# ahtamjidi/3PRE

Measured on AMD Instinct MI355X. Metric: EKF steps/sec (predict+RANSAC+update) at N=500 landmarks; P-update %MFMA peak, higher is better.
Workload: dtype f32

## Files before the change

3pre_amd/_lib.py:

```python
import ctypes as C
import os

import numpy as np

try:
    import torch
except Exception:
    torch = None

_HERE = os.path.dirname(os.path.abspath(__file__))
LIB_PATH = os.environ.get("PRE3_LIB") or os.path.join(_HERE, "lib", "libpre3.so")

if not os.path.exists(LIB_PATH):
    raise ImportError(
        "3pre_amd: %s is missing -- build it with `make -C 3pre_amd/csrc` (or __graft_entry__.build()); "
        "there is no CPU fallback for the HIP path" % LIB_PATH)

lib = C.CDLL(LIB_PATH)
lib.pre3_last_error.restype = C.c_char_p
lib.pre3_version.restype = C.c_char_p
lib.pre3_match_bench_create.restype = C.c_void_p
lib.pre3_match_bench_create_cls.restype = C.c_void_p
lib.pre3_hypothesis_support.argtypes = [C.c_int, C.c_int, C.c_void_p, C.c_void_p, C.c_void_p, C.c_int, C.c_void_p, C.c_int, C.c_void_p, C.c_double, C.c_void_p, C.c_void_p, C.c_void_p]
lib.pre3_step.argtypes = [C.c_void_p, C.c_void_p, C.c_int, C.c_void_p, C.c_void_p, C.c_int, C.c_int, C.c_void_p, C.c_double, C.c_int, C.c_double, C.c_void_p]
# ... 60 lines not shown
lib.pre3_icp.argtypes = [_I, _P, _I, _P, _I, _D, _P, _P, _P, _P, _P, _P]
lib.pre3_icp_limits.argtypes = [_P]
lib.pre3_icp_frames.argtypes = [_P, _P, _I, _D, _P, _P, _P, _P, _P, _P, _P]
lib.pre3_icp_pair_seeded.argtypes = [_P, _P, _D, _U, _U, _I, _D, _P, _P, _P, _P, _P, _P, _P, _P, _P, _P, _P, _P, _P, _P, _P]
lib.pre3_icp_nn_bench.argtypes = [_I, _P, _I, _P, _I, _I, _P]
lib.pre3_icp_cov.argtypes = [_I, _P, _I, _P, _I, _P, _I, _P, _P, _P, _P]
lib.pre3_icp_cov_limits.argtypes = [_P]
lib.pre3_icp_cov_bench.argtypes = [_I, _P, _I, _P, _I, _P, _I, _P, _I, _P]
lib.pre3_predict_icp_pair_seeded.argtypes = [_P, _P, _P, _D, _U, _U, _I, _D, _D, _I, _P, _P, _P, _P, _P, _P]
lib.pre3_icp_pair_cov_seeded.argtypes = [_P, _P, _D, _U, _U, _I, _D, _P, _P, _P, _P, _P, _P, _P, _P, _P, _P, _P, _P, _P, _P, _P, _P, _P, _P, _P]
lib.pre3_epnp.argtypes = [_I, _P, _I, _I, _P, _P, _P]
lib.pre3_pnp_ransac.argtypes = [_I, _P, _I, _I, _P, _P, _I, _P, _D, _P, _P, _P, _P, _P]
lib.pre3_pnp_ransac_seeded.argtypes = [_I, _P, _I, _I, _P, _P, _I, _U, _U, _D, _P, _P, _P, _P, _P, _P]
lib.pre3_pnp_limits.argtypes = [_P]
lib.pre3_vo_pair_pnp_seeded.argtypes = [_P, _P, _D, _U, _U, _P, _I, _P, _P, _P, _P, _P, _P, _P, _P, _P, _P, _P, _P]
lib.pre3_pnp_bench.argtypes = [_I, _P, _I, _I, _P, _P, _I, _U, _U, _D, _I, _P]
lib.pre3_relocalise_seeded.argtypes = [_P, _D, _I, _U, _U, _D, _I, _I, _P, _P, _P, _P]
lib.pre3_reloc_limits.argtypes = [_P]
lib.pre3_pnp_refine.argtypes = [_I, _P, _I, _I, _P, _P, _P, _P, _I, _D, _P]
lib.pre3_pnp_ransac_refined_seeded.argtypes = [_I, _P, _I, _I, _P, _P, _I, _U, _U, _D, _P, _P, _P, _P, _P, _P, _I, _D, _P]
lib.pre3_relocalise_refined_seeded.argtypes = [_P, _D, _I, _U, _U, _D, _I, _I, _I, _D, _I, _P, _P, _P, _P]
lib.pre3_test_downdate.argtypes = [_P, _I, _P, _I]
lib.pre3_test_factor_solve.argtypes = [_P, _I, _P, _P, _P, _I, _I, _P, _P]

F64, F32 = 0, 1
INVDEPTH, CARTESIAN = 0, 1
X_K_K, X_K_KM1 = 0, 1
FAST_MAX_CORNERS, FAST_MAX_ATTEMPTS = 8192, 10


class FastInitResult(C.Structure):
    _fields_ = [("status", C.c_int32), ("attempts", C.c_int32), ("uv", C.c_int32 * 2), ("landmark", C.c_int32), ("pad", C.c_int32), ("rho", C.c_double),
                ("xyz", C.c_double * 3), ("centres", C.c_int32 * 20)]


class Cam(C.Structure):
    _fields_ = [(k, C.c_double) for k in ("f", "Cx", "Cy", "k1", "k2", "nRows", "nCols")]


class Pre3Error(RuntimeError):
    def __init__(self, code, msg):
        super().__init__("libpre3 error %d: %s" % (code, msg))
        self.code = code


def check(rc):
# ... 60 lines not shown
```

3pre_amd/csrc/pre3_api.hip:

```cpp
#include <time.h>
#include <algorithm>
#include <atomic>
#include <immintrin.h>
#include <cmath>
#include <cstdarg>
#include <new>

#include <chrono>
#include "pre3_internal.h"
#include "pre3_test_hooks.h"
#include "pre3_geomdev.h"
#include "pre3_predictu.h"
#include "pre3_predictcv.h"
#include <mutex>
#include "pre3_cholp.h"
#include "pre3_patch.h"
#include "pre3_fast.h"

namespace pre3 {

static thread_local char g_err[512] = "";
void set_error(const char *fmt, ...)
{
    va_list ap; va_start(ap, fmt);
// ... 1534 lines not shown
    c->kt.enabled = false;
    if (mode == 0) c->k9_overlap = false;
    int rc = chol_solve_for_test(c, r_pad, predicted_prior != 0, r);
    c->k9_overlap = ov_was;
    if (rc == PRE3_OK && mode == 1) rc = launch_downdate(c, r, c->W, -1);
    c->kt.enabled = kt_was;
    PRE3_TRY(rc);
    PRE3_TRY(fetch_stats(c));
    if (L_out != nullptr) {
        PRE3_HIP(hipMemcpy(simg.data(), c->Smat, simg.size(), hipMemcpyDeviceToHost));
        for (int i = 0; i < r; ++i)
            for (int j = 0; j < r; ++j) L_out[(size_t)i * r + j] = j <= i ? get(simg, (size_t)i * r_pad + j) : 0.0;
    }
    if (W_out != nullptr) {
        PRE3_HIP(hipMemcpy(wimg.data(), c->W, wimg.size(), hipMemcpyDeviceToHost));
        for (int i = 0; i < r_pad; ++i) {
            for (int j = 0; j < n; ++j) W_out[(size_t)i * (n + 1) + j] = get(wimg, (size_t)i * ldw + j);
            W_out[(size_t)i * (n + 1) + n] = get(wimg, (size_t)i * ldw + c->ld);
        }
    }
    return PRE3_OK;
}

int pre3_match_shard_create_cls(pre3_match_shard **out, int device, int cls, int ND, int K1, const void *L1, int K2_local, const void *L2_local, int k2_offset)
{
    PRE3_CHECK(out != nullptr, PRE3_E_ARG, "pre3_match_shard_create: null output");
    PRE3_TRY(select_device("pre3_match_shard_create", device));
    void *h = match_shard_create(device, cls, ND, K1, L1, K2_local, L2_local, k2_offset);
    if (!h) return PRE3_E_ARG;
    *out = (pre3_match_shard *)h;
    return PRE3_OK;
}
int pre3_match_shard_create(pre3_match_shard **out, int device, int ND, int K1, const uint8_t *L1, int K2_local, const uint8_t *L2_local, int k2_offset)
{
    return pre3_match_shard_create_cls(out, device, 2, ND, K1, L1, K2_local, L2_local, k2_offset);
}
int pre3_match_shard_run(pre3_match_shard *s, void **partial_dev, int *n_doubles) { return s ? match_shard_run(s, partial_dev, n_doubles) : PRE3_E_ARG; }
int pre3_match_shard_merge(pre3_match_shard *s, int G, const void *gathered_dev, double thresh, double *pairs_out, double *score_out, int *M_out)
{
    return s ? match_shard_merge(s, G, gathered_dev, thresh, pairs_out, score_out, M_out) : PRE3_E_ARG;
}
int pre3_match_shard_set_comm(pre3_match_shard *s, pre3_comm *comm) { return s ? match_shard_set_comm(s, comm) : PRE3_E_ARG; }
int pre3_match_shard_match(pre3_match_shard *s, double thresh, double *pairs_out, double *score_out, int *M_out)
{
    return s ? match_shard_match(s, thresh, pairs_out, score_out, M_out) : PRE3_E_ARG;
}
// ... 24 lines not shown
```

3pre_amd/csrc/pre3_geomdev.h:

```cpp
#pragma once
#include "pre3_internal.h"

namespace pre3 {

struct CamD { double f, Cx, Cy, k1, k2, nRows, nCols; };
struct U7 { double v[7]; };
struct VoOut; struct VoPairHeader;
struct PredictUDev { const VoOut *out; const VoPairHeader *hdr; int32_t *err; };
struct VoCov;
struct PnConst {};
struct PnBlock { const double *pn; };
struct PnPair { const VoCov *cov; const VoOut *out; const VoPairHeader *hdr; const double *behind; };
struct IcpCtl;
struct PredictIcpSrc { const VoOut *out; const VoPairHeader *hdr; const VoCov *cov_pair; const IcpCtl *ctl; const double *u_icp, *error; const VoCov *cov_icp;
                       double max_error; int noise; };
struct PredictUIcp { PredictIcpSrc s; int32_t *err; int32_t *taken; };
struct PnIcp { PredictIcpSrc s; const double *behind; };
struct PredictUReloc { const pre3_pnp_result *res; const double *x; int32_t min_support; double *u_out; int32_t *taken_out; };
struct PnReloc { const pre3_pnp_result *res; int32_t min_support; const double *pn; const double *behind; };
struct PredictURelocRef { PredictUReloc b; const pre3_pnp_refine_result *ref; };
struct PnRelocRef { PnReloc b; const pre3_pnp_refine_result *ref; const double *x; int32_t noise; double *pn_out; int32_t *noise_out; };


__device__ inline void d_q2r(const double *q, double *R)
// ... 259 lines not shown
    else active = active && (ic[ii] == 1 && li[ii] == 0);
    const int d = lm_type[ii] == PRE3_INVDEPTH ? 6 : 3;
    const int off = lm_off[ii];
    const int nn = 7 + d;
    double s00 = 0, s01 = 0, s10 = 0, s11 = 0;
    if (active && b < nn) {
        const int ib = b < 7 ? b : off + b - 7;
        const T *prow = P + (size_t)ib * ld;
        double hp0 = 0, hp1 = 0;
#pragma unroll
        for (int a = 0; a < 7; ++a) { double p = (double)prow[a]; hp0 += Hc[14 * ii + a] * p; hp1 += Hc[14 * ii + 7 + a] * p; }
#pragma unroll
        for (int a = 0; a < 6; ++a)
            if (a < d) { double p = (double)prow[off + a]; hp0 += Hl[12 * ii + a] * p; hp1 += Hl[12 * ii + 6 + a] * p; }
        const double h0b = b < 7 ? Hc[14 * ii + b] : Hl[12 * ii + b - 7];
        const double h1b = b < 7 ? Hc[14 * ii + 7 + b] : Hl[12 * ii + 6 + b - 7];
        s00 = hp0 * h0b; s01 = hp0 * h1b; s10 = hp1 * h0b; s11 = hp1 * h1b;
    }
    if (pend_rows > 0 && active) {
        double hc0[7], hc1[7], hl0[6], hl1[6];
#pragma unroll
        for (int a = 0; a < 7; ++a) { hc0[a] = Hc[14 * ii + a]; hc1[a] = Hc[14 * ii + 7 + a]; }
#pragma unroll
        for (int a = 0; a < 6; ++a) { hl0[a] = a < d ? Hl[12 * ii + a] : 0.0; hl1[a] = a < d ? Hl[12 * ii + 6 + a] : 0.0; }
        for (int k = b; k < pend_rows; k += 16) {
            const float *wr = pend_W + (size_t)k * pend_ldw;
            float wp[7], wl[6];
#pragma unroll
            for (int a = 0; a < 7; ++a) wp[a] = wr[a];
#pragma unroll
            for (int a = 0; a < 6; ++a) wl[a] = a < d ? wr[off + a] : 0.f;
            double g0 = 0, g1 = 0;
#pragma unroll
            for (int a = 0; a < 7; ++a) { const double w = (double)wp[a]; g0 += hc0[a] * w; g1 += hc1[a] * w; }
#pragma unroll
            for (int a = 0; a < 6; ++a)
                if (a < d) { const double w = (double)wl[a]; g0 += hl0[a] * w; g1 += hl1[a] * w; }
            s00 -= g0 * g0; s01 -= g0 * g1; s10 -= g1 * g0; s11 -= g1 * g1;
        }
    }
#pragma unroll
    for (int o = 8; o > 0; o >>= 1) {
        s00 += __shfl_xor(s00, o, 16); s01 += __shfl_xor(s01, o, 16);
        s10 += __shfl_xor(s10, o, 16); s11 += __shfl_xor(s11, o, 16);
    }
    if (!valid || b != 0) return;
    if (mode == 0) {
        if (!active) { has_S[i] = 0; return; }
        S[4 * i + 0] = s00 + 1; S[4 * i + 1] = s01; S[4 * i + 2] = s10; S[4 * i + 3] = s11 + 1;
        has_S[i] = 1;
    } else {
        if (!active) return;
        double det = s00 * s11 - s01 * s10;
        double i00 = s11 / det, i01 = -s01 / det, i10 = -s10 / det, i11 = s00 / det;
// ... 9 lines not shown
{
    for (int i0 = threadIdx.x; i0 < ib.n16; i0 += 4 * blockDim.x) {
        int4 v[4];
#pragma unroll
        for (int u = 0; u < 4; ++u) { const int i = i0 + u * blockDim.x; v[u] = i < ib.n16 ? ib.src[i] : int4{ 0, 0, 0, 0 }; }
#pragma unroll
        for (int u = 0; u < 4; ++u) { const int i = i0 + u * blockDim.x; if (i < ib.n16) ib.dst[i] = v[u]; }
    }
    for (int i = threadIdx.x; i < ib.n_clear; i += blockDim.x) ib.clear[i] = 0;
    __syncthreads();
    if (threadIdx.x == 0) { __threadfence_system(); __hip_atomic_store(ib.mail + ib.slot, ib.seq, __ATOMIC_RELEASE, __HIP_MEMORY_SCOPE_SYSTEM); }
}

struct PendW { float *W; int ldw, rows; void *Wp; int nst_total; };
PendW pend_args(const pre3_ctx *c);
int pend_flush(pre3_ctx *c);
struct InnovRide {
    int n_blocks, N, ld, n_clear;
    const int32_t *lm_type, *lm_off, *has_h;
    const void *P; const double *Hc, *Hl;
    double *S; int32_t *has_S, *clear;
    const float *pend_W = nullptr; int pend_ldw = 0, pend_rows = 0;
};
template <typename T>
__device__ __forceinline__ void innov_ride_block(const InnovRide &ir, int blk)
{
    const int gt = blk * blockDim.x + threadIdx.x;
    for (int t = gt; t < ir.n_clear; t += ir.n_blocks * blockDim.x) ir.clear[t] = 0;
    innovation_body<T>(ir.N, ir.lm_type, ir.lm_off, static_cast<const T *>(ir.P), ir.ld, ir.Hc, ir.Hl, ir.has_h, 0, 0.0, nullptr, nullptr, nullptr, nullptr, nullptr,
                       ir.S, ir.has_S, gt, ir.pend_W, ir.pend_ldw, ir.pend_rows);
}

ProjRide make_proj_ride(pre3_ctx *c, int which, int clear_first, int slot, int n_producers);
IcMatchRide ic_match_ride(const pre3_ctx *c);


template <typename ACC> struct Best3 { ACC best, second; int k; };

template <typename ACC> __device__ inline ACC acc_max();
template <> __device__ inline double acc_max<double>() { return INFINITY; }
template <> __device__ inline float acc_max<float>() { return INFINITY; }
template <> __device__ inline int acc_max<int>() { return 0x7fffffff; }

template <typename ACC>
__device__ inline void merge3(ACC &best, ACC &second, int &k, ACC ob, ACC os, int ok)
{
    if (ok < 0) return;
    if (k < 0) { best = ob; second = os; k = ok; return; }
    if (ob < best || (ob == best && ok < k)) {
        ACC ns = os < best ? os : best;
        best = ob; k = ok; second = ns;
    } else {
        ACC ns = ob < second ? ob : second;
// ... 122 lines not shown
```

3pre_amd/csrc/pre3_internal.h:

```cpp
#pragma once
#include <hip/hip_runtime.h>
#include <cstdint>
#include <cstdio>
#include <cstring>
#include <string>
#include <vector>

#include "../../include/pre3.h"
#include "pre3_knobs.h"
#include "pre3_own.h"

namespace pre3 {

void set_error(const char *fmt, ...);

#define PRE3_HIP(call)                                                                         \
    do {                                                                                       \
        hipError_t e_ = (call);                                                                \
        if (e_ != hipSuccess) {                                                                \
            pre3::set_error("%s failed: %s (%s:%d)", #call, hipGetErrorString(e_), __FILE__, __LINE__); \
            return PRE3_E_HIP;                                                                 \
        }                                                                                      \
    } while (0)

// ... 343 lines not shown
struct SrKeypointView { int K, ldf, ND, gate, n_kept; const double *frm, *des; const double *xyz, *rho; const int32_t *keep_idx;
                        int K_in; const double *frm_in, *des_in; bool raw_in_bounds; };
int sr_frame_keypoint_view(pre3_sr_frame *f, SrKeypointView *v);
int sr_frame_pair_work(pre3_sr_frame *f, size_t dev_bytes, size_t pin_bytes, void **dev, void **pin);
int sr_frame_icp_work(pre3_sr_frame *f, size_t dev_bytes, void **dev);
int sr_frame_lend(pre3_sr_frame *f, hipStream_t consumer);
int sr_frame_reclaim(pre3_sr_frame *f, hipStream_t consumer);
int sr_frame_pair_views(const char *who, pre3_sr_frame *prev, pre3_sr_frame *cur, double thresh, SrFrameView *v1, SrFrameView *v2, SrKeypointView *k1,
                        SrKeypointView *k2);
size_t vp_match_part_bytes(int n1, int n2);
int launch_vp_match(int n1, int n2, const double *des1, const double *des2, double thresh, void *part, double *match, void *hdr_dev, hipStream_t st);
int set_descriptors_rows_dev(pre3_ctx *c, int first, int count, const double *des_dev, const int32_t *rows_dev, int n_rows, bool in_bounds);
bool desc_copy_checked(double *dst, const double *src, size_t count);

int launch_book_vis(pre3_ctx *c);

int run_hypothesis_support(int n, const double *xi, const pre3_cam &cam, int n_id, const int32_t *i1, const int32_t *i2, const int32_t *i3,
                           const double *z_id, int n_euc, const int32_t *i4, const double *z_euc, double threshold, int32_t *out_host );

int run_update(pre3_ctx *c, int which_prior, int r, bool dense_R, void *Kt_out_dev , bool prebuilt = false, bool first_done = false,
               bool hp_built = false );
int launch_ell_HP_build_sel(pre3_ctx *c, int nsel, const int32_t *sel_dev , void *dst);
int launch_chol_first_spec(pre3_ctx *c, int nsel_max);
int chol_solve_for_test(pre3_ctx *c, int r_pad, bool predicted_prior, int r);
struct InboxRide;
int launch_ell_HP_build(pre3_ctx *c, void *dst, const int32_t *need = nullptr, int need_tag = 0 ,
                        const InboxRide *ib = nullptr );
int launch_ell_G_hyp(pre3_ctx *c, int k, int lo, int hi, int ldg);
int launch_gather_li(pre3_ctx *c, int nsel , int nsel_max, const int32_t *sel_dev, int ldg);
int launch_select_gather(pre3_ctx *c, int n_draw, int k, int early_exit, int mask_words);
bool select_gather_usable(const pre3_ctx *c);
int launch_ell_HP(pre3_ctx *c, int r, void *dst , bool with_nu);
int launch_ell_G(pre3_ctx *c, int r, const void *HPsrc, void *dst, int ldg, int add_identity, const void *Rdense, bool lower_only = false);
int launch_downdate(pre3_ctx *c, int r, const void *W, int which_prior = -1 ,
                    int planes_rows = 0 );
int launch_fill_w(pre3_ctx *c, int r_pad);
bool hi_fused_usable(const pre3_ctx *c);
int hi_fused_max(const pre3_ctx *c);
int launch_hi_fused(pre3_ctx *c, int32_t seq);

}
```

3pre_amd/csrc/pre3_knobs.h:

```cpp
#pragma once
#include <stdlib.h>

#define PRE3_KNOBS(X) \
     \
    X(tail,              "PRE3_TAIL",              0,  create,  "initial PRE3_OPT_STEP_TAIL: rescue stage + HI update inside the persistent launch; off by default (measured: DESIGN.md section 5d)") \
    X(k9_b3,             "PRE3_K9_B3",             1,  create,  "fp32 contexts, initial PRE3_OPT_K9_BF16X3: three-way bf16 split on the bf16 matrix cores (k_split_w + k_downdate_b3); 0: f32-MFMA down-date, f32 pending updates and trailing tiles") \
    X(pend_hi,           "PRE3_PEND_HI",           0,  create,  "fp32 contexts, initial PRE3_OPT_PEND_HI: the HI update's down-date stays pending across the step boundary (DESIGN.md section 5e); needs 2 .. CP_MAX_NRB + 1 panels of row capacity") \
     \
    X(fuse_jn,           "PRE3_FUSE_JN",           1,  once,    "the rows/cols 3..6 <- Jn pass of a HI update completed at the start of a step rides in that step's prediction launch (0: k_jnorm_P as its own launch; same bits)") \
    X(scan_trace,        "PRE3_SCAN_TRACE",        0,  once,    "pre3_set_scan: host-side phase clock on stderr (event wait, copy + bounds check, positions, enqueue)") \
    X(step_trace,        "PRE3_STEP_TRACE",        0,  present, "host-side stage clock (debug): where the host spends a step, on stderr every 100 steps") \
    X(test_hooks,        "PRE3_TEST_HOOKS",        0,  is1,     "arms pre3_test_stall / pre3_match_shard_test_stall (tests of the communicator's deadline) pre3_test_downdate (K9 alone on the caller's W) and pre3_test_factor_solve (factorisation and solve alone on the caller's S, B, nu); not a performance switch") \
    X(rccl_lib,          "PRE3_RCCL_LIB",          nullptr, text, "path of the RCCL library pre3_comm_* binds (default: librccl.so.1 as already loaded, else from the loader path, else /opt/rocm/lib)") \
     \
    X(inline_g,          "PRE3_INLINE_G",          1,  once,    "RANSAC round: no H*P*H' launch (6.6 us in front of the scoring); the scorer and the LI gather compute their entries with k_ell_G's sum (0: k_ell_G / k_ell_G_hyp as launches; same bits)") \
    X(fuse_rows,         "PRE3_FUSE_ROWS",         1,  once,    "updates of a subset: the ELL rows are built inside the H*P launch (0: k_build_rows + k_ell_HP; same bits)") \
    X(chol_spec0,        "PRE3_CHOL_SPEC0",        1,  once,    "LI update inside pre3_step: the factorisation (fp32: the whole persistent launch; else panel 0) is launched before the host has polled the row count (0: after)") \
    X(pend_max_rows,     "PRE3_PEND_MAX_ROWS",     128, once,   "pending HI rows above which the down-date goes out at once; 128 = 2 NB = never (two pending panels cost the next H*P launch ~19 us more, one ~5; 64 measured 5922 against 5954 steps/s)") \
    X(ride_rescue,       "PRE3_RIDE_RESCUE",       1,  once,    "the rescue's projection rides in the LI update's K9 launch (0: projection + gate as one launch of their own, A/B)") \
    X(ride_proj,         "PRE3_RIDE_PROJ",         1,  once,    "the projection of every landmark rides in the prediction's launch (0: its own launch, A/B)") \
    X(ride_innov,        "PRE3_RIDE_INNOV",        1,  once,    "S_i (which also clears last frame's inlier flags) rides in the H*P launch of the RANSAC stage (0: its own launch)") \
     \
    X(gate_ride,         "PRE3_GATE_RIDE",         1,  once,    "the rescue's chi2 gate rides in the Jnorm pass's launch (0: a launch of its own behind it, rounds 3-4)") \
    X(select_gather,     "PRE3_SELECT_GATHER",     1,  once,    "pre3_step: the selection stage rides in the LI gather's launch (k_select_gather); 0: k_ransac_select + k_gather_li (same bits)") \
    X(select_gather_lds, "PRE3_SELECT_GATHER_LDS", 1,  once,    "k_select_gather in its LDS-staged form where the rows of H*P fit in 55 KB (0: the form gathering from global memory; same bits)") \
     \
    X(k9_wt,             "PRE3_K9_WT",             1,  once,    "k_downdate_b3 and the one-tile K9 store P write-through (neutral at N = 2000: 1851 vs 1855 us; part of the HI update's down-date at N = 500)") \
    X(hp_mb,             "PRE3_HP_MB",             1,  once,    "H*P build: several measurements per workgroup (k_ell_HP_build_mb; shares the pose rows' loads, no faster: a ~7.7 us latency chain); 0: one per workgroup (k_ell_HP_build; same bits)") \
    X(pend_mb,           "PRE3_PEND_MB",           4,  once,    "measurements per workgroup of the pending H*P form: 4 (17.1 -> 16.5 us with their landmark rows gathered two at a time); 8 halves the loads of W~ but leaves 156 workgroups for 256 CUs (18.7 us), 2 doubles them (21.5 us)") \
    X(chol_pro_b3,       "PRE3_CHOL_PRO_B3",       1,  once,    "with the bf16-split down-date: pending updates / trailing tiles of the per-panel factorisation from bf16 planes (0: f32 MFMA; the planes of W then come from riders)") \
    X(chol_early,        "PRE3_CHOL_EARLY",        1,  once,    "per-panel factorisation: the last panel of an update whose row count is no multiple of 64 skips the chain steps behind its last real sub-panel (0: all of them; same bits)") \
    X(chol_trail_split,  "PRE3_CHOL_TRAIL_SPLIT",  4,  once,    "trailing updates with more than this x 2 x #CUs tiles go out as a launch of their own (no LDS, 8 workgroups per CU); 0: never") \
    X(chol_trail_p,      "PRE3_CHOL_TRAIL_P",      4,  once,    "panels per trailing sweep, clamped to 1 .. 4 (1: the one-panel sweep; same bits)") \
    X(chol_trail_t128,   "PRE3_CHOL_TRAIL_T128",   2,  once,    "the sweep's W part in 128 x 128 super-tiles with the operands staged through LDS (k_chol_trail_b3l); 0: 64 x 64 tiles (k_chol_trail_b3; same bits)") \
    X(k9_wgs,            "PRE3_K9_WGS",            3,  once,    "f32/f64 MFMA down-date, persistent form: workgroups per CU") \
// ... 42 lines not shown
```

3pre_amd/csrc/pre3_test_hooks.h:

```cpp
#pragma once
#include "../../include/pre3.h"
#ifdef __cplusplus
extern "C" {
#endif
PRE3_API int pre3_test_stall(pre3_ctx *ctx, int release);
PRE3_API int pre3_match_shard_test_stall(pre3_match_shard *s, int release);
PRE3_API int pre3_test_downdate(pre3_ctx *ctx, int r, const double *W, int launches);
PRE3_API int pre3_test_factor_solve(pre3_ctx *ctx, int r, const double *S, const double *B, const double *nu, int mode, int predicted_prior, double *L_out, double *W_out);
PRE3_API int pre3_test_live_blocks(int64_t out[4]);
#ifdef __cplusplus
}
#endif
```

3pre_amd/csrc/pre3_update.hip:

```cpp
#include <algorithm>
#include <atomic>
#include <cstdlib>

#include "pre3_internal.h"
#include "pre3_geomdev.h"
#include "pre3_chain.h"
#include "pre3_chain_async.h"
#ifndef PRE3_CHAIN_ASYNC_F64
#define PRE3_CHAIN_ASYNC_F64 0
#endif
#ifndef PRE3_CHAIN_ASYNC
#define PRE3_CHAIN_ASYNC 1
#endif
#include "pre3_cholp.h"

namespace pre3 {

template <typename T>
__global__ __launch_bounds__(256) void k_ell_HP(int r, int r_pad, const int32_t *__restrict__ row_col, const T *__restrict__ row_val,
                                                const double *__restrict__ row_nu, const T *__restrict__ P, int ld, T *__restrict__ dst,
                                                int ldw, int with_nu)
{
    int a = blockIdx.y;
    int j = blockIdx.x * blockDim.x + threadIdx.x;
// ... 5 lines not shown
#pragma unroll
            for (int t = 0; t < ELLW; ++t) {
                T v = row_val[a * ELLW + t];
                int c = row_col[a * ELLW + t];
                s += v * P[(size_t)c * ld + j];
            }
            out = s;
        } else if (j == ld && with_nu) {
            out = (T)row_nu[a];
        }
    }
    dst[(size_t)a * ldw + j] = out;
}

template <typename T>
__global__ __launch_bounds__(256) void k_ell_HP_build(int m, int r_pad, const int32_t *__restrict__ meas, const int32_t *__restrict__ lm_type,
                                                      const int32_t *__restrict__ lm_off, const double *__restrict__ Hc,
                                                      const double *__restrict__ Hl, const double *__restrict__ z, const double *__restrict__ h,
                                                      int32_t *__restrict__ row_col, T *__restrict__ row_val, double *__restrict__ row_nu,
                                                      const T *__restrict__ P, int ld, T *__restrict__ dst, int ldw, const int32_t *__restrict__ need, int need_tag,
                                                      int ny_build, InnovRide ir, const int32_t *__restrict__ sel = nullptr, InboxRide ib = InboxRide{})
{
    if (ib.n16 > 0 && blockIdx.y == gridDim.y - 1) { if (blockIdx.x == 0) inbox_pull_block(ib); return; }
    if ((int)blockIdx.y >= ny_build) { innov_ride_block<T>(ir, ((int)blockIdx.y - ny_build) * gridDim.x + blockIdx.x); return; }
    if (need != nullptr && (int)blockIdx.y < m && need[blockIdx.y] != need_tag) return;
    typedef T v4_t __attribute__((ext_vector_type(4)));
    const int sIdx = blockIdx.y;
    const int j = (blockIdx.x * blockDim.x + threadIdx.x) * 4;
    if (2 * sIdx >= r_pad) return;
    v4_t out0 = { (T)0, (T)0, (T)0, (T)0 }, out1 = out0;
    if (sIdx < m) {
        const int i = meas[sel ? sel[sIdx] : sIdx];
        const int d = lm_type[i] == PRE3_INVDEPTH ? 6 : 3, off = lm_off[i];
        T v0[13], v1[13]; int cc[13];
#pragma unroll
        for (int t = 0; t < 7; ++t) { cc[t] = t; v0[t] = (T)Hc[14 * i + t]; v1[t] = (T)Hc[14 * i + 7 + t]; }
#pragma unroll
        for (int t = 0; t < 6; ++t) { cc[7 + t] = t < d ? off + t : 0; v0[7 + t] = t < d ? (T)Hl[12 * i + t] : (T)0; v1[7 + t] = t < d ? (T)Hl[12 * i + 6 + t] : (T)0; }
        const double nu0 = z[2 * i] - h[2 * i], nu1 = z[2 * i + 1] - h[2 * i + 1];
        if (blockIdx.x == 0) {
            if (threadIdx.x < 2 * ELLW) {
                const int t = threadIdx.x & (ELLW - 1), c = threadIdx.x >> 4;
                int cv = 0; T vt = (T)0;
#pragma unroll
                for (int u = 0; u < 13; ++u) if (u == t) { cv = cc[u]; vt = c ? v1[u] : v0[u]; }
                row_col[(2 * sIdx + c) * ELLW + t] = cv; row_val[(2 * sIdx + c) * ELLW + t] = vt;
            }
// ... 66 lines not shown
        }
    }
    const int j = (blockIdx.x * blockDim.x + tid) * 4;
    const int prow = PEND ? (pw.rows < PEND_MAX ? pw.rows : PEND_MAX) : 0;
    int any = 0;
#pragma unroll
    for (int mi = 0; mi < MB; ++mi) any |= state[mi] == 2;
    constexpr int GB = PEND ? 2 : (MB < 4 ? MB : 4);
    v4_t pp[7], lp[GB][6];
    const bool inside = j < ld;
    auto load_lp = [&](const int h) {
#pragma unroll
        for (int u = 0; u < GB; ++u)
            if (state[h + u] == 2) {
#pragma unroll
                for (int t = 0; t < 6; ++t) lp[u][t] = *reinterpret_cast<const v4_t *>(P + (size_t)ccs[h + u][7 + t] * ld + j);
            }
    };
    if (inside && any) {
#pragma unroll
        for (int t = 0; t < 7; ++t) pp[t] = *reinterpret_cast<const v4_t *>(P + (size_t)t * ld + j);
        load_lp(0);
    }
    constexpr int KB = PRE3_PEND_KB;
    const bool corr = PEND && prow > 0 && (int)(blockIdx.x * blockDim.x * 4) < ld;
    const bool corr_t = corr && inside && any;
    v4_t wa[KB], wb[KB];
    auto loadw = [&](v4_t (&w)[KB], const int k0) {
#pragma unroll
        for (int u = 0; u < KB; ++u) { const int k = k0 + u < prow ? k0 + u : prow - 1; w[u] = *reinterpret_cast<const v4_t *>(reinterpret_cast<const T *>(pw.W) + (size_t)k * pw.ldw + j); }
    };
    v4_t out[MB][2];
    auto applyw = [&](const v4_t (&w)[KB], const int k0) {
#pragma unroll
        for (int u = 0; u < KB; ++u) {
            if (k0 + u < prow) {
#pragma unroll
                for (int mi = 0; mi < MB; ++mi) { out[mi][0] -= (T)gp[(k0 + u) * (2 * MB) + 2 * mi] * w[u]; out[mi][1] -= (T)gp[(k0 + u) * (2 * MB) + 2 * mi + 1] * w[u]; }
            }
        }
    };
    if (corr) {
        for (int e = tid; e < MB * prow; e += 256) {
            const int mi = e % MB, k = e / MB;
            float g0 = 0.f, g1 = 0.f;
            if (state[mi] == 2) {
                const float *wr = pw.W + (size_t)k * pw.ldw;
#pragma unroll
                for (int t = 0; t < 13; ++t) { const float wv = wr[ccs[mi][t]]; g0 += (float)cv[mi][0][t] * wv; g1 += (float)cv[mi][1][t] * wv; }
            }
            gp[k * (2 * MB) + 2 * mi] = g0; gp[k * (2 * MB) + 2 * mi + 1] = g1;
        }
        __syncthreads();
    }
    if (j >= ldw) return;
#pragma unroll
    for (int h = 0; h < MB; h += GB) {
        if (h > 0 && inside && any) load_lp(h);
#pragma unroll
        for (int u = 0; u < GB; ++u) {
            const int mi = h + u;
            v4_t out0 = { (T)0, (T)0, (T)0, (T)0 }, out1 = out0;
            if (state[mi] == 2) {
                if (inside) {
#pragma unroll
                    for (int t = 0; t < 7; ++t) { out0 += cv[mi][0][t] * pp[t]; out1 += cv[mi][1][t] * pp[t]; }
#pragma unroll
                    for (int t = 0; t < 6; ++t) { out0 += cv[mi][0][7 + t] * lp[u][t]; out1 += cv[mi][1][7 + t] * lp[u][t]; }
                } else if (j == ld) {
                    out0[0] = (T)nus[mi][0]; out1[0] = (T)nus[mi][1];
                }
            }
            out[mi][0] = out0; out[mi][1] = out1;
        }
    }
    if (corr_t) {
        asm volatile("" ::: "memory");
        loadw(wa, 0);
        for (int k0 = 0; k0 < prow; k0 += 2 * KB) {
            if (k0 + KB < prow) loadw(wb, k0 + KB);
            applyw(wa, k0);
            if (k0 + 2 * KB < prow) loadw(wa, k0 + 2 * KB);
            if (k0 + KB < prow) applyw(wb, k0 + KB);
        }
    }
#pragma unroll
    for (int mi = 0; mi < MB; ++mi) {
        const int sIdx = s0 + mi;
        if (state[mi] == 0) continue;
        *reinterpret_cast<v4_t *>(dst + (size_t)(2 * sIdx) * ldw + j) = out[mi][0];
        *reinterpret_cast<v4_t *>(dst + (size_t)(2 * sIdx + 1) * ldw + j) = out[mi][1];
    }
}

template <typename T>
__global__ __launch_bounds__(64) void k_ell_G(int r, int r_pad, const int32_t *__restrict__ row_col, const T *__restrict__ row_val,
                                              const T *__restrict__ HP, int ldw, T *__restrict__ dst, int ldg, int add_identity,
                                              const T *__restrict__ Rd, int lower_only)
{
    int a = blockIdx.y;
    int b = blockIdx.x * blockDim.x + threadIdx.x;
    if (b >= r_pad || a >= r_pad) return;
    T out;
    if (lower_only && (int)(blockIdx.x * blockDim.x) > a) {
        out = (T)0;
    } else if (a < r && b < r) {
// ... 1761 lines not shown
    if (knob::hp_mb() > 0 && need == nullptr) {
        constexpr int MBF = 4, MBD = 2;
        const int mbf = pw.rows > 0 ? (knob::pend_mb() == 8 ? 8 : 4) : MBF;
        auto kd = k_ell_HP_build_mb<double, MBD>; auto kf = pw.rows > 0 ? (mbf == 8 ? k_ell_HP_build_mb<float, 8, true> : k_ell_HP_build_mb<float, 4, true>) : k_ell_HP_build_mb<float, MBF, false>;
        const int nyg = c->dtype == PRE3_F32 ? ceil_div(ny, mbf) : ceil_div(ny, MBD);
        dim3 g(gx, nyg + (ir.n_blocks ? ir.n_blocks / gx : 0) + ib_rows), b(256);
        DISPATCH_T(c,
            hipLaunchKernelGGL(kd, g, b, 0, c->stream, c->m, r_pad, c->meas, c->lm.type, c->lm.off, c->lm.Hc, c->lm.Hl, c->lm.z, c->lm.h,
                               c->row_col, (double *)c->row_val, c->row_nu, (const double *)c->P, c->ld, (double *)dst, c->ldw, need, need_tag, nyg, ir, (const int32_t *)nullptr, ib, PendW{}),
            hipLaunchKernelGGL(kf, g, b, 0, c->stream, c->m, r_pad, c->meas, c->lm.type, c->lm.off, c->lm.Hc, c->lm.Hl, c->lm.z, c->lm.h,
                               c->row_col, (float *)c->row_val, c->row_nu, (const float *)c->P, c->ld, (float *)dst, c->ldw, need, need_tag, nyg, ir, (const int32_t *)nullptr, ib, pw));
        PRE3_HIP(hipGetLastError());
        if (ir.n_blocks) { c->out.innovation_rode = true; c->innovated = true; }
        return PRE3_OK;
    }
    dim3 g(gx, ny + (ir.n_blocks ? ir.n_blocks / gx : 0) + ib_rows), b(256);
    DISPATCH_T(c,
        hipLaunchKernelGGL(k_ell_HP_build<double>, g, b, 0, c->stream, c->m, r_pad, c->meas, c->lm.type, c->lm.off, c->lm.Hc, c->lm.Hl, c->lm.z, c->lm.h,
                           c->row_col, (double *)c->row_val, c->row_nu, (const double *)c->P, c->ld, (double *)dst, c->ldw, need, need_tag, ny, ir, (const int32_t *)nullptr, ib),
        hipLaunchKernelGGL(k_ell_HP_build<float>, g, b, 0, c->stream, c->m, r_pad, c->meas, c->lm.type, c->lm.off, c->lm.Hc, c->lm.Hl, c->lm.z, c->lm.h,
                           c->row_col, (float *)c->row_val, c->row_nu, (const float *)c->P, c->ld, (float *)dst, c->ldw, need, need_tag, ny, ir, (const int32_t *)nullptr, ib));
    PRE3_HIP(hipGetLastError());
    if (ir.n_blocks) { c->out.innovation_rode = true; c->innovated = true; }
    return PRE3_OK;
}

int launch_ell_G(pre3_ctx *c, int r, const void *HPsrc, void *dst, int ldg, int add_identity, const void *Rdense, bool lower_only)
{
    int r_pad = round_up(r, NB);
    dim3 g(ceil_div(r_pad, 64), r_pad), b(64);
    DISPATCH_T(c,
        hipLaunchKernelGGL(k_ell_G<double>, g, b, 0, c->stream, r, r_pad, c->row_col, (const double *)c->row_val, (const double *)HPsrc,
                           c->ldw, (double *)dst, ldg, add_identity, (const double *)Rdense, lower_only ? 1 : 0),
        hipLaunchKernelGGL(k_ell_G<float>, g, b, 0, c->stream, r, r_pad, c->row_col, (const float *)c->row_val, (const float *)HPsrc,
                           c->ldw, (float *)dst, ldg, add_identity, (const float *)Rdense, lower_only ? 1 : 0));
    PRE3_HIP(hipGetLastError());
    return PRE3_OK;
}

int launch_ell_G_hyp(pre3_ctx *c, int k, int lo, int hi, int ldg)
{
    if (hi <= lo) return PRE3_OK;
    dim3 g(ceil_div((hi - lo) * k * (2 * k + 1), 256)), b(256);
    DISPATCH_T(c,
        hipLaunchKernelGGL(k_ell_G_hyp<double>, g, b, 0, c->stream, c->hyp, k, lo, hi, c->row_col, (const double *)c->row_val, (const double *)c->HP, c->ldw, (double *)c->G, ldg),
        hipLaunchKernelGGL(k_ell_G_hyp<float>, g, b, 0, c->stream, c->hyp, k, lo, hi, c->row_col, (const float *)c->row_val, (const float *)c->HP, c->ldw, (float *)c->G, ldg));
// ... 374 lines not shown
```

3pre_amd/ekf.py:

```python
import ctypes as C

import numpy as np

from . import _lib
from ._lib import Cam, Pre3Error, addr, check, dptr, f64, i32, lib

CHI2INV_2_95 = 5.9915


def _cam(cam):
    if isinstance(cam, dict):
        cam = [cam[k] for k in ("f", "Cx", "Cy", "k1", "k2", "nRows", "nCols")]
    return Cam(*[float(v) for v in cam])


class EkfFilter:

    def __init__(self, cam, lm_type, dtype="f32", device=0, max_hyp=1000, max_landmarks=None, std_z=1.0):
        lm_type = i32(lm_type)
        self.N = int(lm_type.shape[0])
        self.dtype = {"f64": _lib.F64, "f32": _lib.F32}[dtype]
        self.std_z = float(std_z)
        self._ctx = C.c_void_p()
        check(lib.pre3_create(C.byref(self._ctx), int(device), self.dtype, int(max_landmarks or max(self.N, 1)), int(max_hyp)))
# ... 665 lines not shown
            return dict(best=int(st[0]), iters=int(st[1]), n_hyp=int(st[2]), max_support=int(st[3]))
        sup = np.zeros(n_draw, np.int32)
        li = np.zeros(max(self.m, 1), np.int32)
        check(lib.pre3_ransac_sharded(self._ctx, n_draw, k, dptr(hyp), C.c_double(float(threshold)), int(bool(early_exit)), dptr(sup), dptr(li), dptr(st)))
        return dict(support=sup, li_mask=li[:self.m], best=int(st[0]), iters=int(st[1]), n_hyp=int(st[2]), max_support=int(st[3]))

    def test_stall(self, release):
        check(lib.pre3_test_stall(self._ctx, int(release)))

    def test_downdate(self, W, launches=1):
        W = f64(W)
        if W.ndim != 2 or W.shape[1] != self.n:
            raise ValueError("test_downdate: W must be r x %d" % self.n)
        check(lib.pre3_test_downdate(self._ctx, int(W.shape[0]), dptr(W), int(launches)))

    def test_factor_solve(self, S, B, nu, mode=0, predicted_prior=False):
        S, B, nu = f64(S), f64(B), f64(nu)
        r = S.shape[0]
        if S.ndim != 2 or S.shape != (r, r) or B.shape != (r, self.n) or nu.shape != (r,):
            raise ValueError("test_factor_solve: S must be r x r, B r x %d, nu r" % self.n)
        L, W = np.zeros((r, r)), np.zeros(((r + 63) // 64 * 64, self.n + 1))
        check(lib.pre3_test_factor_solve(self._ctx, int(r), dptr(S), dptr(B), dptr(nu), int(mode), int(bool(predicted_prior)), dptr(L), dptr(W)))
        return L, W

    def ransac_export(self, n_draw, support_ptr, mask_ptr):
        check(lib.pre3_ransac_export(self._ctx, int(n_draw), C.c_void_p(support_ptr), C.c_void_p(mask_ptr)))

    def ransac_import(self, n_draw, support_ptr, mask_ptr):
        check(lib.pre3_ransac_import(self._ctx, int(n_draw), C.c_void_p(support_ptr), C.c_void_p(mask_ptr)))

    def ekf_update_li_inliers(self):
        check(lib.pre3_update_li(self._ctx))

    def rescue_hi_inliers(self, chi2=CHI2INV_2_95):
        hi = np.zeros(max(self.m, 1), np.int32)
        check(lib.pre3_rescue(self._ctx, C.c_double(chi2), dptr(hi)))
        return hi[:self.m]

    def ekf_update_hi_inliers(self):
        check(lib.pre3_update_hi(self._ctx))

    def ekf_update_all(self):
        check(lib.pre3_update_all(self._ctx))

    def set_flags(self, li=None, hi=None):
        li = None if li is None else i32(li)
# ... 189 lines not shown
```

Before: 7405.

## Software-pipeline pending-row correction in fp32 HP build; vectorize landmark row loads

The pending-W correction loop in the fp32 H*P build kernel now splits into whole-chunk iterations, which use a new applyw_whole path, and a partial tail. applyw_whole preloads the G coefficients a fixed distance ahead of the FMAs, with scheduling barriers between stages, and halves the chunk size when MB is 8 to limit register pressure. The innovation-ride blocks inside the build kernel no longer run the pending correction (MAY_PEND=false), and the landmark W rows are read as one packed 6-float load. A test hook is also added to run the build launch alone. The risks are higher register use and a possible correctness change if the ride blocks still needed the pending rows.

```diff
diff --git a/3pre_amd/_lib.py b/3pre_amd/_lib.py
--- a/3pre_amd/_lib.py
+++ b/3pre_amd/_lib.py
@@ -106,6 +106,8 @@
 lib.pre3_relocalise_refined_seeded.argtypes = [_P, _D, _I, _U, _U, _D, _I, _I, _I, _D, _I, _P, _P, _P, _P]
 lib.pre3_test_downdate.argtypes = [_P, _I, _P, _I]
 lib.pre3_test_factor_solve.argtypes = [_P, _I, _P, _P, _P, _I, _I, _P, _P]
+if hasattr(lib, "pre3_test_hp_pending"):
+    lib.pre3_test_hp_pending.argtypes = [_P, _I, _P, _P, _P]
 
 F64, F32 = 0, 1
 INVDEPTH, CARTESIAN = 0, 1
diff --git a/3pre_amd/csrc/pre3_api.hip b/3pre_amd/csrc/pre3_api.hip
--- a/3pre_amd/csrc/pre3_api.hip
+++ b/3pre_amd/csrc/pre3_api.hip
@@ -1580,6 +1580,44 @@
     return PRE3_OK;
 }
 
+int pre3_test_hp_pending(pre3_ctx *c, int rows, const double *Wt, double *HP_out, double *Si_out)
+{
+    PRE3_CHECK(knob::test_hooks(), PRE3_E_STATE, "pre3_test_hp_pending: test hooks are off (PRE3_TEST_HOOKS=1 enables them)");
+    PRE3_CHECK(c != nullptr && (rows == 0 || Wt != nullptr) && HP_out != nullptr && Si_out != nullptr, PRE3_E_ARG, "pre3_test_hp_pending: null pointer");
+    PRE3_CHECK(rows >= 0 && rows <= 2 * NB, PRE3_E_ARG, "pre3_test_hp_pending: rows must be 0 .. %d", 2 * NB);
+    PRE3_CHECK(c->dtype == PRE3_F32 && knob::hp_mb() > 0, PRE3_E_STATE, "pre3_test_hp_pending: the pending form is the fp32 PRE3_HP_MB launch");
+    PRE3_CHECK(c->n > 0 && c->N > 0 && c->projected, PRE3_E_STATE, "pre3_test_hp_pending: no map/state set, or pre3_project has not run");
+    PRE3_CHECK(c->m >= 1 && round_up(2 * c->m, NB) <= c->rcap, PRE3_E_STATE, "pre3_test_hp_pending: no measurements installed");
+    for (size_t i = 0; i < (size_t)rows * c->n; ++i) PRE3_CHECK(std::isfinite((float)Wt[i]), PRE3_E_ARG, "pre3_test_hp_pending: Wt has a non-finite entry");
+    EntryScope scope(c, Entry::reader); PRE3_TRY(scope.rc);
+    const int n = c->n, N = c->N, ldw = c->ldw, r = 2 * c->m, r_pad = round_up(r, NB);
+    std::vector<float> wimg((size_t)(rows ? rows : 1) * ldw, 0.f), hp((size_t)r_pad * ldw);
+    for (int k = 0; k < rows; ++k)
+        for (int j = 0; j < n; ++j) wimg[(size_t)k * ldw + j] = (float)Wt[(size_t)k * n + j];
+    BlockList tmp;
+    float *d_w = nullptr, *d_hp = nullptr; double *d_S = nullptr; int32_t *d_has = nullptr;
+    PRE3_TRY(tmp.dev(&d_w, sizeof(float) * wimg.size(), Zero::sync()));
+    PRE3_TRY(tmp.dev(&d_hp, sizeof(float) * hp.size(), Zero::sync()));
+    PRE3_TRY(tmp.dev(&d_S, sizeof(double) * 4 * N, Zero::sync()));
+    PRE3_TRY(tmp.dev(&d_has, sizeof(int32_t) * N, Zero::sync()));
+    PRE3_TRY(stream_drain(c, __func__));
+    PRE3_HIP(hipMemcpy(d_w, wimg.data(), sizeof(float) * wimg.size(), hipMemcpyHostToDevice));
+    c->hp_all_valid = false; c->g_valid = false;
+    PRE3_TRY(hp_pending_for_test(c, d_w, rows, d_hp, d_S, d_has));
+    PRE3_TRY(stream_drain(c, __func__));
+    std::vector<double> S4((size_t)4 * N); std::vector<int32_t> has(N);
+    PRE3_HIP(hipMemcpy(hp.data(), d_hp, sizeof(float) * hp.size(), hipMemcpyDeviceToHost));
+    PRE3_HIP(hipMemcpy(S4.data(), d_S, sizeof(double) * 4 * N, hipMemcpyDeviceToHost));
+    PRE3_HIP(hipMemcpy(has.data(), d_has, sizeof(int32_t) * N, hipMemcpyDeviceToHost));
+    for (int a = 0; a < r; ++a) {
+        for (int j = 0; j < n; ++j) HP_out[(size_t)a * (n + 1) + j] = (double)hp[(size_t)a * ldw + j];
+        HP_out[(size_t)a * (n + 1) + n] = (double)hp[(size_t)a * ldw + c->ld];
+    }
+    for (int i = 0; i < N; ++i)
+        for (int e = 0; e < 4; ++e) Si_out[4 * i + e] = has[i] ? S4[4 * i + e] : std::nan("");
+    return PRE3_OK;
+}
+
 int pre3_match_shard_create_cls(pre3_match_shard **out, int device, int cls, int ND, int K1, const void *L1, int K2_local, const void *L2_local, int k2_offset)
 {
     PRE3_CHECK(out != nullptr, PRE3_E_ARG, "pre3_match_shard_create: null output");
diff --git a/3pre_amd/csrc/pre3_geomdev.h b/3pre_amd/csrc/pre3_geomdev.h
--- a/3pre_amd/csrc/pre3_geomdev.h
+++ b/3pre_amd/csrc/pre3_geomdev.h
@@ -305,14 +305,16 @@
 #pragma unroll
         for (int a = 0; a < 7; ++a) { hc0[a] = Hc[14 * ii + a]; hc1[a] = Hc[14 * ii + 7 + a]; }
 #pragma unroll
-        for (int a = 0; a < 6; ++a) { hl0[a] = a < d ? Hl[12 * ii + a] : 0.0; hl1[a] = a < d ? Hl[12 * ii + 6 + a] : 0.0; }
+        for (int a = 0; a < 6; ++a) { const double l0 = Hl[12 * ii + a], l1 = Hl[12 * ii + 6 + a]; hl0[a] = a < d ? l0 : 0.0; hl1[a] = a < d ? l1 : 0.0; }
+        struct __attribute__((packed, aligned(4))) PRow6 { float v[6]; };
         for (int k = b; k < pend_rows; k += 16) {
             const float *wr = pend_W + (size_t)k * pend_ldw;
             float wp[7], wl[6];
+            const PRow6 lv = *reinterpret_cast<const PRow6 *>(wr + off);
 #pragma unroll
             for (int a = 0; a < 7; ++a) wp[a] = wr[a];
 #pragma unroll
-            for (int a = 0; a < 6; ++a) wl[a] = a < d ? wr[off + a] : 0.f;
+            for (int a = 0; a < 6; ++a) wl[a] = a < d ? lv.v[a] : 0.f;
             double g0 = 0, g1 = 0;
 #pragma unroll
             for (int a = 0; a < 7; ++a) { const double w = (double)wp[a]; g0 += hc0[a] * w; g1 += hc1[a] * w; }
@@ -368,13 +370,13 @@
     double *S; int32_t *has_S, *clear;
     const float *pend_W = nullptr; int pend_ldw = 0, pend_rows = 0;
 };
-template <typename T>
+template <typename T, bool MAY_PEND = true >
 __device__ __forceinline__ void innov_ride_block(const InnovRide &ir, int blk)
 {
     const int gt = blk * blockDim.x + threadIdx.x;
     for (int t = gt; t < ir.n_clear; t += ir.n_blocks * blockDim.x) ir.clear[t] = 0;
     innovation_body<T>(ir.N, ir.lm_type, ir.lm_off, static_cast<const T *>(ir.P), ir.ld, ir.Hc, ir.Hl, ir.has_h, 0, 0.0, nullptr, nullptr, nullptr, nullptr, nullptr,
-                       ir.S, ir.has_S, gt, ir.pend_W, ir.pend_ldw, ir.pend_rows);
+                       ir.S, ir.has_S, gt, MAY_PEND ? ir.pend_W : nullptr, MAY_PEND ? ir.pend_ldw : 0, MAY_PEND ? ir.pend_rows : 0);
 }
 
 ProjRide make_proj_ride(pre3_ctx *c, int which, int clear_first, int slot, int n_producers);
diff --git a/3pre_amd/csrc/pre3_internal.h b/3pre_amd/csrc/pre3_internal.h
--- a/3pre_amd/csrc/pre3_internal.h
+++ b/3pre_amd/csrc/pre3_internal.h
@@ -389,6 +389,7 @@
                bool hp_built = false );
 int launch_ell_HP_build_sel(pre3_ctx *c, int nsel, const int32_t *sel_dev , void *dst);
 int launch_chol_first_spec(pre3_ctx *c, int nsel_max);
+int hp_pending_for_test(pre3_ctx *c, const float *Wt, int rows, float *dst, double *S, int32_t *has_S);
 int chol_solve_for_test(pre3_ctx *c, int r_pad, bool predicted_prior, int r);
 struct InboxRide;
 int launch_ell_HP_build(pre3_ctx *c, void *dst, const int32_t *need = nullptr, int need_tag = 0 ,
diff --git a/3pre_amd/csrc/pre3_knobs.h b/3pre_amd/csrc/pre3_knobs.h
--- a/3pre_amd/csrc/pre3_knobs.h
+++ b/3pre_amd/csrc/pre3_knobs.h
@@ -10,7 +10,7 @@
     X(fuse_jn,           "PRE3_FUSE_JN",           1,  once,    "the rows/cols 3..6 <- Jn pass of a HI update completed at the start of a step rides in that step's prediction launch (0: k_jnorm_P as its own launch; same bits)") \
     X(scan_trace,        "PRE3_SCAN_TRACE",        0,  once,    "pre3_set_scan: host-side phase clock on stderr (event wait, copy + bounds check, positions, enqueue)") \
     X(step_trace,        "PRE3_STEP_TRACE",        0,  present, "host-side stage clock (debug): where the host spends a step, on stderr every 100 steps") \
-    X(test_hooks,        "PRE3_TEST_HOOKS",        0,  is1,     "arms pre3_test_stall / pre3_match_shard_test_stall (tests of the communicator's deadline) pre3_test_downdate (K9 alone on the caller's W) and pre3_test_factor_solve (factorisation and solve alone on the caller's S, B, nu); not a performance switch") \
+    X(test_hooks,        "PRE3_TEST_HOOKS",        0,  is1,     "arms pre3_test_stall / pre3_match_shard_test_stall (tests of the communicator's deadline) pre3_test_downdate (K9 alone on the caller's W) pre3_test_factor_solve (factorisation and solve alone on the caller's S, B, nu) and pre3_test_hp_pending (the H*P build launch alone on the caller's pending rows); not a performance switch") \
     X(rccl_lib,          "PRE3_RCCL_LIB",          nullptr, text, "path of the RCCL library pre3_comm_* binds (default: librccl.so.1 as already loaded, else from the loader path, else /opt/rocm/lib)") \
      \
     X(inline_g,          "PRE3_INLINE_G",          1,  once,    "RANSAC round: no H*P*H' launch (6.6 us in front of the scoring); the scorer and the LI gather compute their entries with k_ell_G's sum (0: k_ell_G / k_ell_G_hyp as launches; same bits)") \
diff --git a/3pre_amd/csrc/pre3_test_hooks.h b/3pre_amd/csrc/pre3_test_hooks.h
--- a/3pre_amd/csrc/pre3_test_hooks.h
+++ b/3pre_amd/csrc/pre3_test_hooks.h
@@ -7,6 +7,7 @@
 PRE3_API int pre3_match_shard_test_stall(pre3_match_shard *s, int release);
 PRE3_API int pre3_test_downdate(pre3_ctx *ctx, int r, const double *W, int launches);
 PRE3_API int pre3_test_factor_solve(pre3_ctx *ctx, int r, const double *S, const double *B, const double *nu, int mode, int predicted_prior, double *L_out, double *W_out);
+PRE3_API int pre3_test_hp_pending(pre3_ctx *ctx, int rows, const double *Wt, double *HP_out, double *Si_out);
 PRE3_API int pre3_test_live_blocks(int64_t out[4]);
 #ifdef __cplusplus
 }
diff --git a/3pre_amd/csrc/pre3_update.hip b/3pre_amd/csrc/pre3_update.hip
--- a/3pre_amd/csrc/pre3_update.hip
+++ b/3pre_amd/csrc/pre3_update.hip
@@ -51,7 +51,7 @@
                                                       int ny_build, InnovRide ir, const int32_t *__restrict__ sel = nullptr, InboxRide ib = InboxRide{})
 {
     if (ib.n16 > 0 && blockIdx.y == gridDim.y - 1) { if (blockIdx.x == 0) inbox_pull_block(ib); return; }
-    if ((int)blockIdx.y >= ny_build) { innov_ride_block<T>(ir, ((int)blockIdx.y - ny_build) * gridDim.x + blockIdx.x); return; }
+    if ((int)blockIdx.y >= ny_build) { innov_ride_block<T, false>(ir, ((int)blockIdx.y - ny_build) * gridDim.x + blockIdx.x); return; }
     if (need != nullptr && (int)blockIdx.y < m && need[blockIdx.y] != need_tag) return;
     typedef T v4_t __attribute__((ext_vector_type(4)));
     const int sIdx = blockIdx.y;
@@ -164,16 +164,39 @@
         for (int t = 0; t < 7; ++t) pp[t] = *reinterpret_cast<const v4_t *>(P + (size_t)t * ld + j);
         load_lp(0);
     }
-    constexpr int KB = PRE3_PEND_KB;
+    constexpr int KB = MB == 8 ? PRE3_PEND_KB / 2 : PRE3_PEND_KB;
     const bool corr = PEND && prow > 0 && (int)(blockIdx.x * blockDim.x * 4) < ld;
     const bool corr_t = corr && inside && any;
     v4_t wa[KB], wb[KB];
     auto loadw = [&](v4_t (&w)[KB], const int k0) {
 #pragma unroll
-        for (int u = 0; u < KB; ++u) { const int k = k0 + u < prow ? k0 + u : prow - 1; w[u] = *reinterpret_cast<const v4_t *>(reinterpret_cast<const T *>(pw.W) + (size_t)k * pw.ldw + j); }
+        for (int u = 0; u < KB; ++u) {
+            const int k = k0 + u < prow ? k0 + u : prow - 1;
+            w[u] = *reinterpret_cast<const v4_t *>(reinterpret_cast<const T *>(pw.W) + (size_t)k * pw.ldw + (unsigned)j);
+        }
     };
     v4_t out[MB][2];
-    auto applyw = [&](const v4_t (&w)[KB], const int k0) {
+    constexpr int GD = 2;
+    auto applyw_whole = [&](const v4_t (&w)[KB], const int k0) {
+        if constexpr (PEND) {
+            constexpr int UR = MB / 4, NU = KB * UR;
+            float g[NU][8];
+#pragma unroll
+            for (int q = 0; q < NU + GD; ++q) {
+                if (q < NU) {
+#pragma unroll
+                    for (int e = 0; e < 8; ++e) g[q][e] = gp[(k0 + q / UR) * (2 * MB) + 8 * (q % UR) + e];
+                }
+                if (q >= GD) {
+                    const int p = q - GD, u = p / UR, m0 = 4 * (p % UR);
+#pragma unroll
+                    for (int mi = 0; mi < 4; ++mi) { out[m0 + mi][0] -= (T)g[p][2 * mi] * w[u]; out[m0 + mi][1] -= (T)g[p][2 * mi + 1] * w[u]; }
+                }
+                __builtin_amdgcn_sched_barrier(0);
+            }
+        }
+    };
+    auto applyw_part = [&](const v4_t (&w)[KB], const int k0) {
 #pragma unroll
         for (int u = 0; u < KB; ++u) {
             if (k0 + u < prow) {
@@ -219,11 +242,17 @@
     if (corr_t) {
         asm volatile("" ::: "memory");
         loadw(wa, 0);
-        for (int k0 = 0; k0 < prow; k0 += 2 * KB) {
+        int k0 = 0;
+        for (; k0 + 2 * KB <= prow; k0 += 2 * KB) {
+            loadw(wb, k0 + KB);
+            applyw_whole(wa, k0);
+            loadw(wa, k0 + 2 * KB);
+            applyw_whole(wb, k0 + KB);
+        }
+        if (k0 < prow) {
             if (k0 + KB < prow) loadw(wb, k0 + KB);
-            applyw(wa, k0);
-            if (k0 + 2 * KB < prow) loadw(wa, k0 + 2 * KB);
-            if (k0 + KB < prow) applyw(wb, k0 + KB);
+            if (MB == 4 && k0 + KB <= prow) applyw_whole(wa, k0); else applyw_part(wa, k0);
+            if (k0 + KB < prow) applyw_part(wb, k0 + KB);
         }
     }
 #pragma unroll
@@ -2031,6 +2060,24 @@
                            c->row_col, (float *)c->row_val, c->row_nu, (const float *)c->P, c->ld, (float *)dst, c->ldw, need, need_tag, ny, ir, (const int32_t *)nullptr, ib));
     PRE3_HIP(hipGetLastError());
     if (ir.n_blocks) { c->out.innovation_rode = true; c->innovated = true; }
+    return PRE3_OK;
+}
+
+int hp_pending_for_test(pre3_ctx *c, const float *Wt, int rows, float *dst, double *S, int32_t *has_S)
+{
+    const int r_pad = round_up(2 * c->m, NB);
+    const int gx = ceil_div(c->ldw / 4, 256), ny = r_pad / 2;
+    const int nb = ceil_div(c->N * 16, 256), ir_rows = ceil_div(nb, gx);
+    InnovRide ir{ ir_rows * gx, c->N, c->ld, 0, c->lm.type, c->lm.off, c->lm.has_h, c->P, c->lm.Hc, c->lm.Hl, S, has_S, nullptr };
+    PendW pw{};
+    if (rows > 0) { pw = PendW{ const_cast<float *>(Wt), c->ldw, rows, nullptr, 0 }; ir.pend_W = Wt; ir.pend_ldw = c->ldw; ir.pend_rows = rows; }
+    const int mbf = rows > 0 ? (knob::pend_mb() == 8 ? 8 : 4) : 4;
+    auto kf = rows > 0 ? (mbf == 8 ? k_ell_HP_build_mb<float, 8, true> : k_ell_HP_build_mb<float, 4, true>) : k_ell_HP_build_mb<float, 4, false>;
+    const int nyg = ceil_div(ny, mbf);
+    dim3 g(gx, nyg + ir.n_blocks / gx), b(256);
+    hipLaunchKernelGGL(kf, g, b, 0, c->stream, c->m, r_pad, c->meas, c->lm.type, c->lm.off, c->lm.Hc, c->lm.Hl, c->lm.z, c->lm.h,
+                       c->row_col, (float *)c->row_val, c->row_nu, (const float *)c->P, c->ld, dst, c->ldw, (const int32_t *)nullptr, 0, nyg, ir, (const int32_t *)nullptr, InboxRide{}, pw);
+    PRE3_HIP(hipGetLastError());
     return PRE3_OK;
 }
 
diff --git a/3pre_amd/ekf.py b/3pre_amd/ekf.py
--- a/3pre_amd/ekf.py
+++ b/3pre_amd/ekf.py
@@ -711,6 +711,12 @@
         L, W = np.zeros((r, r)), np.zeros(((r + 63) // 64 * 64, self.n + 1))
         check(lib.pre3_test_factor_solve(self._ctx, int(r), dptr(S), dptr(B), dptr(nu), int(mode), int(bool(predicted_prior)), dptr(L), dptr(W)))
         return L, W
+
+    def test_hp_pending(self, Wt):
+        Wt = f64(Wt).reshape(-1, self.n) if np.size(Wt) else np.zeros((0, self.n))
+        HP, Si = np.zeros((2 * self.m, self.n + 1)), np.zeros((self.N, 2, 2))
+        check(lib.pre3_test_hp_pending(self._ctx, int(Wt.shape[0]), dptr(Wt) if Wt.shape[0] else None, dptr(HP), dptr(Si)))
+        return HP, Si
 
     def ransac_export(self, n_draw, support_ptr, mask_ptr):
         check(lib.pre3_ransac_export(self._ctx, int(n_draw), C.c_void_p(support_ptr), C.c_void_p(mask_ptr)))
```

After: 7401 (median of 2 runs). Within noise of the previous version (-0.1%).
